# DeepMed-Lab-ECNU/BCP

Measured on AMD Instinct MI355X. Metric: training volumes/sec (LA 112x112x80 V-Net, BCP self-training step), higher is better.
Workload: dtype f32 (fp16x2 split operands); 1 GPU; LA 3D V-Net BCP self-train step, per-GPU batch 4 (2 labeled), 112x112x80 patches, SGD m0.9 wd1e-4, EMA 0.99 (BASELINE.json configs[1]); global_batch=4, parallelism=dp1

## Files before the change

bcp_amd/csrc/conv3.hip:

```cpp
#include "conv3_defs.h"
#include "../../include/bcp_hip.h"
#include <cstdlib>
#include <cstdio>

namespace bcp {

template <int KD, int TD, int TH, int TW, int NT, int WT>
__global__ __launch_bounds__(256) void k_conv3_mfma(const float* __restrict__ X, const float* __restrict__ Wp,
                                                    const float* __restrict__ bias, float* __restrict__ Y, ConvDims cd,
                                                    int accumulate, StatsArg st) {
  using TL = Tile<KD, TD, TH, TW>;
  constexpr int MT = TL::MT, T = TL::T, CT = NT * 16;
  constexpr int S = T / WT;
  static_assert(T % WT == 0, "WT must divide the tap count");
  constexpr int NBUF = (S > 1) ? 2 : 1;
  constexpr int WSTAGE4 = WT * 4 * CT;
  constexpr int NW4 = (WSTAGE4 + 255) / 256;
  constexpr int NACC = (MT * NT == 1) ? 2 : 1;

  HIP_DYNAMIC_SHARED(float4, smem4)
  float* smem = reinterpret_cast<float*>(smem4);
  float* Xs = smem;
  float* Ws = smem + TL::HV * XS;
  double* Ss = reinterpret_cast<double*>(Ws + NBUF * WSTAGE4 * 4);
// ... 781 lines not shown
    const bool twin = (d.dgrad & 0x800) != 0 && di > 0;
    d.dgrad &= 1;
    const int nb = d.N16 >> 4, k0 = (u / nb) * 16, n0 = (u % nb) * 16, T = d.T;
    const int row0 = d.dgrad ? k0 : n0, in0 = d.dgrad ? n0 : k0;
    for (int q = threadIdx.x; q < 256 * T; q += 256) {
      const int r = q / (16 * T), rem = q - r * 16 * T;
      const int in = rem / T, t = rem - in * T;
      float v = 0.f;
      if (row0 + r < d.Cout && in0 + in < d.Cin) v = d.w[((long long)(row0 + r) * d.Cin + in0 + in) * T + t];
      tile[q] = v;
    }
    __syncthreads();
    if (sec & 1)
    for (int q = threadIdx.x; q < 256 * T; q += 256) {
      const int k4 = q & 3, nn = (q >> 2) & 15, kq = (q >> 6) & 3, t = q >> 8;
      const int kk = kq * 4 + k4;
      const float v = d.dgrad ? tile[(kk * 16 + nn) * T + (T - 1 - t)] : tile[(nn * 16 + kk) * T + t];
      d.wp[(((long long)t * (d.K16 >> 2) + (k0 >> 2) + kq) * d.N16 + n0 + nn) * 4 + k4] = v;
    }
    {
      const int TP = (T + 1) / 2, ch = k0 >> 4;
      unsigned* wb = reinterpret_cast<unsigned*>(d.wp + (long long)T * d.K16 * d.N16);
      if (sec & 2)
      for (int q = threadIdx.x; q < TP * 16 * 16; q += 256) {
        const int j2 = q & 15, nn = (q >> 4) & 15, tp = q >> 8;
        const int t = 2 * tp + (j2 >> 3), kk = (j2 * 2) & 15;
        float v0 = 0.f, v1 = 0.f;
        if (t < T) {
          v0 = d.dgrad ? tile[(kk * 16 + nn) * T + (T - 1 - t)] : tile[(nn * 16 + kk) * T + t];
          v1 = d.dgrad ? tile[((kk + 1) * 16 + nn) * T + (T - 1 - t)] : tile[(nn * 16 + kk + 1) * T + t];
        }
        unsigned* o = wb + ((((((long long)ch * TP + tp) * 3) * d.N16 + n0 + nn) * 32 + j2 * 2) >> 1);
        const long long ps = ((long long)d.N16 * 32) >> 1;
        unsigned h = cvt_pk_bf16(v0, v1);
        o[0] = h;
        v0 -= __uint_as_float(h << 16); v1 -= __uint_as_float(h & 0xffff0000u);
        h = cvt_pk_bf16(v0, v1);
        o[ps] = h;
        v0 -= __uint_as_float(h << 16); v1 -= __uint_as_float(h & 0xffff0000u);
        o[2 * ps] = cvt_pk_bf16(v0, v1);
      }
      float* hdr = d.wp + pack_off_hdr(T, d.K16, d.N16);
      const float* hsrc = hdr;
      if (twin) { const PackDesc t = descs[di - 1]; hsrc = t.wp + pack_off_hdr(t.T, t.K16, t.N16); }
      float amax = 0.f;
#pragma unroll
      for (int b = 0; b < 16; ++b) amax = fmaxf(amax, hsrc[1 + b]);
      const float sc = f16_scale(amax);
      if (u == 0 && threadIdx.x == 0) hdr[0] = amax;
      unsigned* wh = reinterpret_cast<unsigned*>(d.wp + pack_off_f16(T, d.K16, d.N16));
      if (sec & 4)
      for (int q = threadIdx.x; q < TP * 16 * 16; q += 256) {
        const int j2 = q & 15, nn = (q >> 4) & 15, tp = q >> 8;
        const int t = 2 * tp + (j2 >> 3), kk = (j2 * 2) & 15;
        float v0 = 0.f, v1 = 0.f;
        if (t < T) {
          v0 = d.dgrad ? tile[(kk * 16 + nn) * T + (T - 1 - t)] : tile[(nn * 16 + kk) * T + t];
          v1 = d.dgrad ? tile[((kk + 1) * 16 + nn) * T + (T - 1 - t)] : tile[(nn * 16 + kk + 1) * T + t];
        }
        v0 *= sc; v1 *= sc;
        unsigned* o = wh + ((((((long long)ch * TP + tp) * 2) * d.N16 + n0 + nn) * 32 + j2 * 2) >> 1);
        const long long ps = ((long long)d.N16 * 32) >> 1;
        const unsigned h = cvt_pk_f16(v0, v1);
        o[0] = h;
        o[ps] = cvt_pk_f16(v0 - f16lo_to_f32(h), v1 - f16hi_to_f32(h));
      }
    }
    __syncthreads();
  }
}

struct C1Norm {
  const float* stats;
  const float* da;
  const float* c1c2;
  const uint8_t* elem_mask;
  float elem_scale;
  int act, G;
  float* amax;
  const unsigned long long* mask_seed;
  float p_keep;
};

template <int KD, int TD, int TH, int TW, int EPI = 0>
__global__ __launch_bounds__(256) void k_conv3_c1(const float* __restrict__ X, const float* __restrict__ w ,
                                                  const float* __restrict__ bias, float* __restrict__ Y, ConvDims cd, int n_tiles,
                                                  int tiles_per_block, StatsArg st, C1Norm nm) {
  using TL = Tile<KD, TD, TH, TW>;
  constexpr int T = TL::T, MT = TL::MT, KS = (T + 3) / 4;
  __shared__ __attribute__((aligned(16))) float Xs[TL::HV];
  __shared__ double Ss[4 * 16 * 2];
  __shared__ __attribute__((aligned(16))) float Ys[EPI == 5 ? TL::M * 16 : 4];
  static_assert(EPI != 5 || (TL::M == 256 && T <= 32 && MT == 4), "EPI 5: four waves x 64 voxels, two 16-tap MFMA row tiles");
  const int lane = threadIdx.x & 63, wave = threadIdx.x >> 6;
  const int li = lane & 15, lg = lane >> 4;
  int aoff[2] = {0, 0};
  f32x4 wacc[2] = {(f32x4){0.f, 0.f, 0.f, 0.f}, (f32x4){0.f, 0.f, 0.f, 0.f}};
  if (EPI == 5) {
#pragma unroll
    for (int tt = 0; tt < 2; ++tt) aoff[tt] = (tt * 16 + li < T) ? TL::tapoff(tt * 16 + li) : 0;
  }
  float wv[KS];
  int toff[KS];
#pragma unroll
  for (int ks = 0; ks < KS; ++ks) {
    const int tap = ks * 4 + lg;
    wv[ks] = tap < T ? w[li * T + tap] : 0.f;
    toff[ks] = tap < T ? TL::tapoff(tap) : 0;
  }
  float4 bv = make_float4(0.f, 0.f, 0.f, 0.f);
  if (bias) bv = ld4(bias + lg * 4);
  double s1[4] = {0, 0, 0, 0}, s2[4] = {0, 0, 0, 0};
  float amax_o = 0.f;
  unsigned mseed_lo = 0, mseed_hi = 0;
  if (EPI >= 2 && nm.mask_seed) { const unsigned long long s_ = *nm.mask_seed; mseed_lo = (unsigned)s_; mseed_hi = (unsigned)(s_ >> 32); }
  const bool has_mask = EPI >= 2 && (nm.elem_mask != nullptr || nm.mask_seed != nullptr);
  const int t_begin = blockIdx.x * tiles_per_block;
  int t_end = t_begin + tiles_per_block;
  if (t_end > n_tiles) t_end = n_tiles;
  float mu[4] = {0, 0, 0, 0}, rs[4] = {1, 1, 1, 1}, sc[4] = {1, 1, 1, 1}, sh[4] = {0, 0, 0, 0}, k1[4] = {0, 0, 0, 0}, k2[4] = {0, 0, 0, 0};
  if (EPI >= 2) {
    const int g = t_begin / st.tiles_per_group;
    const long long GC = (long long)nm.G * 16, o = (long long)g * 16 + lg * 4;
#pragma unroll
    for (int r = 0; r < 4; ++r) {
      mu[r] = nm.stats[o + r]; rs[r] = nm.stats[GC + o + r]; sc[r] = nm.stats[2 * GC + o + r]; sh[r] = nm.stats[3 * GC + o + r];
      if (EPI >= 4) { k1[r] = nm.c1c2[o + r]; k2[r] = nm.c1c2[GC + o + r]; }
    }
  }
  constexpr bool PRE = KD == 3;
  constexpr int NPRE = (TL::HV + 255) / 256;
  float pre[NPRE];
  auto fetch = [&](int tile) __attribute__((always_inline)) {
    int n, d0, h0, w0;
    tile_origin(cd, tile, TD, TH, TW, n, d0, h0, w0);
#pragma unroll
    for (int i = 0; i < NPRE; ++i) {
      const int q = threadIdx.x + i * 256;
      const int hw = q % TL::HW, hh = (q / TL::HW) % TL::HH, hd = q / (TL::HW * TL::HH);
      const int d = d0 - TL::PD + hd, h = h0 - 1 + hh, wq = w0 - 1 + hw;
      float v = 0.f;
      if (q < TL::HV && (unsigned)d < (unsigned)cd.D && (unsigned)h < (unsigned)cd.H && (unsigned)wq < (unsigned)cd.W)
        v = X[(((long long)n * cd.D + d) * cd.H + h) * cd.W + wq];
      pre[i] = v;
    }
  };
  if (PRE && t_begin < t_end) fetch(t_begin);
  for (int tile = t_begin; tile < t_end; ++tile) {
    int n, d0, h0, w0;
    tile_origin(cd, tile, TD, TH, TW, n, d0, h0, w0);
    if (tile > t_begin) __syncthreads();
    if (!PRE) fetch(tile);
#pragma unroll
    for (int i = 0; i < NPRE; ++i)
      if (threadIdx.x + i * 256 < TL::HV) Xs[threadIdx.x + i * 256] = pre[i];
    __syncthreads();
    if (PRE && tile + 1 < t_end) fetch(tile + 1);
    const bool full = d0 + TD <= cd.D && h0 + TH <= cd.H && w0 + TW <= cd.W;
#pragma unroll
    for (int mt = 0; mt < MT; ++mt) {
      const int m = (wave * MT + mt) * 16 + li;
      const int vo = TL::voff(m);
      const int tw = m % TW, th = (m / TW) % TH, td = m / (TW * TH);
      const int d = d0 + td, h = h0 + th, wq = w0 + tw;
      const bool ok = full || (d < cd.D && h < cd.H && wq < cd.W);
      const long long e = ((((long long)n * cd.D + d) * cd.H + h) * cd.W + wq) * 16 + lg * 4;
      float4 dav = make_float4(0.f, 0.f, 0.f, 0.f);
      uchar4 m4 = make_uchar4(1, 1, 1, 1);
      if (EPI >= 3 && ok) dav = ld4(nm.da + e);
      if (has_mask && ok) m4 = nm.mask_seed ? bern_keep4(e, mseed_lo, mseed_hi, nm.p_keep) : *reinterpret_cast<const uchar4*>(nm.elem_mask + e);
      f32x4 acc = (f32x4){0.f, 0.f, 0.f, 0.f};
#pragma unroll
      for (int ks = 0; ks < KS; ++ks) acc = __builtin_amdgcn_mfma_f32_16x16x4f32(wv[ks], Xs[vo + toff[ks]], acc, 0, 0, 0);
      float4 dyl = make_float4(0.f, 0.f, 0.f, 0.f);
      if (ok) {
        const float yv[4] = {acc[0] + bv.x, acc[1] + bv.y, acc[2] + bv.z, acc[3] + bv.w};
        if (EPI == 0) st4(Y + e, make_float4(yv[0], yv[1], yv[2], yv[3]));
        if (EPI <= 1) {
          if (st.partial) {
#pragma unroll
            for (int r = 0; r < 4; ++r) { s1[r] += (double)yv[r]; s2[r] += (double)yv[r] * (double)yv[r]; }
          }
        } else {
          const float ms[4] = {m4.x ? nm.elem_scale : 0.f, m4.y ? nm.elem_scale : 0.f, m4.z ? nm.elem_scale : 0.f, m4.w ? nm.elem_scale : 0.f};
          const float dd[4] = {dav.x, dav.y, dav.z, dav.w};
          float o[4];
#pragma unroll
          for (int r = 0; r < 4; ++r) {
            const float z = (yv[r] - mu[r]) * sc[r] + sh[r];
            if (EPI == 2) {
              o[r] = act_fwd(z, nm.act);
              if (has_mask) o[r] *= ms[r];
              const float t = fabsf(o[r]);
              amax_o = (t > amax_o || t != t) ? t : amax_o;
            } else {
              const float cs = has_mask ? ms[r] : 1.f;
              const float dz = dd[r] * cs * act_grad(z, nm.act);
              const float xh = (yv[r] - mu[r]) * rs[r];
              if (EPI == 3) { s1[r] += (double)dz; s2[r] += (double)dz * (double)xh; }
              else o[r] = sc[r] * (dz - k1[r] - xh * k2[r]);
            }
          }
          if (EPI == 2 || EPI == 4) st4(Y + e, make_float4(o[0], o[1], o[2], o[3]));
          if (EPI == 5) dyl = make_float4(o[0], o[1], o[2], o[3]);
        }
      }
      if (EPI == 5) st4(Ys + m * 16 + lg * 4, dyl);
    }
    if (EPI == 5) {
      __syncthreads();
#pragma unroll 4
      for (int ks = 0; ks < 16; ++ks) {
        const int v = wave * 64 + ks * 4 + lg;
        const int vo = TL::voff(v);
        const float b = Ys[v * 16 + li];
        wacc[0] = __builtin_amdgcn_mfma_f32_16x16x4f32(Xs[vo + aoff[0]], b, wacc[0], 0, 0, 0);
        wacc[1] = __builtin_amdgcn_mfma_f32_16x16x4f32(Xs[vo + aoff[1]], b, wacc[1], 0, 0, 0);
      }
    }
  }
  if (EPI == 5) {
    __syncthreads();
    float* red = Ys;
#pragma unroll
    for (int tt = 0; tt < 2; ++tt)
#pragma unroll
      for (int r = 0; r < 4; ++r) red[(wave * 32 + tt * 16 + lg * 4 + r) * 16 + li] = wacc[tt][r];
    __syncthreads();
    for (int o = threadIdx.x; o < T * 16; o += 256)
      Y[(long long)blockIdx.x * T * 16 + o] = (red[o] + red[512 + o]) + (red[1024 + o] + red[1536 + o]);
  }
  if (st.partial) {
#pragma unroll
    for (int r = 0; r < 4; ++r) {
      double a = s1[r], b = s2[r];
#pragma unroll
      for (int o = 1; o < 16; o <<= 1) { a += __shfl_xor(a, o); b += __shfl_xor(b, o); }
      if (li == 0) { Ss[(wave * 16 + lg * 4 + r) * 2] = a; Ss[(wave * 16 + lg * 4 + r) * 2 + 1] = b; }
    }
    __syncthreads();
    if (threadIdx.x < 16) {
      const int c = threadIdx.x;
      double a = 0.0, b = 0.0;
#pragma unroll
      for (int wv_ = 0; wv_ < 4; ++wv_) { a += Ss[(wv_ * 16 + c) * 2]; b += Ss[(wv_ * 16 + c) * 2 + 1]; }
      const int gg = t_begin / st.tiles_per_group, row = (t_begin % st.tiles_per_group) / tiles_per_block;
      double* dst = st.partial + (((long long)gg * st.rows + row) * 16 + c) * 2;
      dst[0] = a; dst[1] = b;
    }
  }
  if (EPI == 2 && nm.amax) { __syncthreads(); block_amax_publish(amax_o, nm.amax); }
}

template <int KD, int TD, int TH, int TW>
__global__ __launch_bounds__(256) void k_conv3_c1_wgrad(const float* __restrict__ X, const float* __restrict__ dY,
                                                        float* __restrict__ partial, ConvDims cd, int tiles_total,
                                                        int tiles_per_group) {
  using TL = Tile<KD, TD, TH, TW>;
  constexpr int T = TL::T, M = TL::M;
  static_assert(M == 256 && T <= 32, "four waves x 64 voxels, two 16-tap MFMA row tiles");
  constexpr int NXS = (TL::HV + 255) / 256;
  __shared__ __attribute__((aligned(16))) float Xs[TL::HV];
  __shared__ __attribute__((aligned(16))) float Ys[M * 16];
  const int lane = threadIdx.x & 63, wave = threadIdx.x >> 6;
  const int li = lane & 15, lg = lane >> 4;
  const int grp = blockIdx.x;
  int t_end = (grp + 1) * tiles_per_group;
  if (t_end > tiles_total) t_end = tiles_total;
  int tile = grp * tiles_per_group;
  if (tile >= t_end) return;

  int aoff[2];
#pragma unroll
  for (int tt = 0; tt < 2; ++tt) aoff[tt] = (tt * 16 + li < T) ? TL::tapoff(tt * 16 + li) : 0;
  f32x4 acc[2] = {(f32x4){0.f, 0.f, 0.f, 0.f}, (f32x4){0.f, 0.f, 0.f, 0.f}};

  float px[NXS];
  float4 py[4];
  auto fetch = [&](int tl) {
    int n, d0, h0, w0;
    tile_origin(cd, tl, TD, TH, TW, n, d0, h0, w0);
#pragma unroll
    for (int u = 0; u < NXS; ++u) {
      const int q = threadIdx.x + u * 256;
      float v = 0.f;
      if (q < TL::HV) {
        const int hw = q % TL::HW, hh = (q / TL::HW) % TL::HH, hd = q / (TL::HW * TL::HH);
        const int d = d0 - TL::PD + hd, h = h0 - 1 + hh, wq = w0 - 1 + hw;
        if ((unsigned)d < (unsigned)cd.D && (unsigned)h < (unsigned)cd.H && (unsigned)wq < (unsigned)cd.W)
          v = X[(((long long)n * cd.D + d) * cd.H + h) * cd.W + wq];
      }
      px[u] = v;
    }
#pragma unroll
    for (int u = 0; u < 4; ++u) {
      const int q = threadIdx.x + u * 256;
      const int m = q >> 2, c4 = q & 3;
      const int tw = m % TW, th = (m / TW) % TH, td = m / (TW * TH);
      const int d = d0 + td, h = h0 + th, wq = w0 + tw;
      float4 v = make_float4(0.f, 0.f, 0.f, 0.f);
      if (d < cd.D && h < cd.H && wq < cd.W) v = ld4(dY + ((((long long)n * cd.D + d) * cd.H + h) * cd.W + wq) * 16 + c4 * 4);
      py[u] = v;
    }
  };
  auto stash = [&]() {
#pragma unroll
    for (int u = 0; u < NXS; ++u) {
      const int q = threadIdx.x + u * 256;
      if (q < TL::HV) Xs[q] = px[u];
    }
#pragma unroll
    for (int u = 0; u < 4; ++u) st4(Ys + (threadIdx.x + u * 256) * 4, py[u]);
  };
// ... 534 lines not shown
    default: c1_launch<0>(KD, grid, s, x, w, bias, y, cd, tiles, tpb, st, nm); break;
  }
  return st.rows;
}

extern "C" int bcp_conv3_c1_fwd(const float* x, const float* w, const float* bias, float* y, int N, int D, int H, int W, int KD,
                                void* stream) {
  BCP_REQUIRE(x && w && y, "bcp_conv3_c1_fwd: null pointer");
  BCP_REQUIRE((KD == 1 && D == 1) || KD == 3, "bcp_conv3_c1_fwd: bad KD/D");
  BCP_REQUIRE(aligned16(y) && (!bias || aligned16(bias)), "bcp_conv3_c1_fwd: y / bias must be 16-B aligned");
  c1_fwd_impl(x, w, bias, y, N, D, H, W, KD, nullptr, 0, false, (hipStream_t)stream);
  BCP_CHECK_LAUNCH("bcp_conv3_c1_fwd");
  return BCP_OK;
}

extern "C" int bcp_conv3_c1_stat_rows(int N, int D, int H, int W, int KD, int groups) {
  if (groups < 1 || N < 1 || D < 1 || H < 1 || W < 1 || !((KD == 1 && D == 1) || KD == 3)) return 0;
  return c1_fwd_impl(nullptr, nullptr, nullptr, nullptr, N, D, H, W, KD, nullptr, groups, true, nullptr);
}

extern "C" int bcp_conv3_c1_fwd_stats(const float* x, const float* w, const float* bias, float* y, int N, int D, int H, int W, int KD,
                                      double* stat_partial, int groups, void* stream) {
  BCP_REQUIRE(x && w && y && stat_partial && groups >= 1, "bcp_conv3_c1_fwd_stats: null pointer / bad groups");
  BCP_REQUIRE((KD == 1 && D == 1) || KD == 3, "bcp_conv3_c1_fwd_stats: bad KD/D");
  BCP_REQUIRE(aligned16(y) && (!bias || aligned16(bias)), "bcp_conv3_c1_fwd_stats: y / bias must be 16-B aligned");
  const int rows = c1_fwd_impl(x, w, bias, y, N, D, H, W, KD, stat_partial, groups, false, (hipStream_t)stream);
  BCP_REQUIRE(rows > 0, "bcp_conv3_c1_fwd_stats: fused statistics unavailable (N %% groups != 0): check bcp_conv3_c1_stat_rows first");
  BCP_CHECK_LAUNCH("bcp_conv3_c1_fwd_stats");
  return BCP_OK;
}

namespace bcp {
void norm_fwd_finalize_launch(const double* partial, int nb, int G, int C, long long rows_per_group, const float* gamma, const float* beta,
                              float* running_mean, float* running_var, float momentum, float eps, float* stats, hipStream_t s, float* amax_clear_or_null);
void norm_bwd_finalize_launch(const double* partial, int nb, int G, int C, long long rows_per_group, float* dgamma, float* dbeta, int accumulate,
                              float* c1c2raw, hipStream_t s, float* amax_clear_or_null);
}

extern "C" size_t bcp_conv3_c1_norm_workspace_bytes(int N, int D, int H, int W, int KD, int groups) {
  const int rows = bcp_conv3_c1_stat_rows(N, D, H, W, KD, groups);
  return rows > 0 ? (size_t)groups * rows * 16 * 2 * sizeof(double) + (size_t)4 * groups * 16 * sizeof(float) : 0;
}

extern "C" int bcp_conv3_c1_norm_fwd(const float* x, const float* w, const float* bias, int N, int D, int H, int W, int KD, int groups,
                                     const float* gamma, const float* beta, float* running_mean, float* running_var, float momentum, float eps,
                                     int act, const uint8_t* elem_mask, float elem_scale, const unsigned long long* mask_seed, float mask_p_keep,
                                     float* stats, void* workspace, float* out, float* amax_out_or_null, void* stream) {
  BCP_REQUIRE(x && w && stats && workspace && out && groups >= 1, "bcp_conv3_c1_norm_fwd: null pointer / bad groups");
  BCP_REQUIRE((KD == 1 && D == 1) || KD == 3, "bcp_conv3_c1_norm_fwd: bad KD/D");
  BCP_REQUIRE(aligned16(out) && aligned16(stats) && (!bias || aligned16(bias)), "bcp_conv3_c1_norm_fwd: alignment");
  hipStream_t s = (hipStream_t)stream;
  double* partial = reinterpret_cast<double*>(workspace);
  const int rows = c1_fwd_impl(x, w, bias, nullptr, N, D, H, W, KD, partial, groups, false, s, 1);
  BCP_REQUIRE(rows > 0, "bcp_conv3_c1_norm_fwd: the groups must be whole samples (N %% groups == 0)");
  norm_fwd_finalize_launch(partial, rows, groups, 16, (long long)N / groups * D * H * W, gamma, beta, running_mean, running_var, momentum, eps, stats, s,
                           amax_out_or_null);
  const C1Norm nm{stats, nullptr, nullptr, elem_mask, elem_scale, act, groups, amax_out_or_null, mask_seed, mask_p_keep};
  c1_fwd_impl(x, w, bias, out, N, D, H, W, KD, nullptr, groups, false, s, 2, &nm);
  BCP_CHECK_LAUNCH("bcp_conv3_c1_norm_fwd");
  return BCP_OK;
}

extern "C" int bcp_conv3_c1_norm_bwd(const float* x, const float* w, const float* bias, const float* da, int N, int D, int H, int W, int KD,
                                     int groups, const float* stats, int act, const uint8_t* elem_mask, float elem_scale,
                                     const unsigned long long* mask_seed, float mask_p_keep, float* dgamma,
                                     float* dbeta, int accumulate, void* workspace, float* dy, void* stream) {
  BCP_REQUIRE(x && w && da && stats && workspace && dy && groups >= 1, "bcp_conv3_c1_norm_bwd: null pointer / bad groups");
  BCP_REQUIRE((KD == 1 && D == 1) || KD == 3, "bcp_conv3_c1_norm_bwd: bad KD/D");
  BCP_REQUIRE(aligned16(da) && aligned16(dy) && (!bias || aligned16(bias)), "bcp_conv3_c1_norm_bwd: alignment");
  BCP_REQUIRE((dgamma == nullptr) == (dbeta == nullptr), "bcp_conv3_c1_norm_bwd: dgamma and dbeta come together");
  hipStream_t s = (hipStream_t)stream;
  double* partial = reinterpret_cast<double*>(workspace);
  const int rows0 = bcp_conv3_c1_stat_rows(N, D, H, W, KD, groups);
  BCP_REQUIRE(rows0 > 0, "bcp_conv3_c1_norm_bwd: the groups must be whole samples (N %% groups == 0)");
  float* c1c2raw = reinterpret_cast<float*>(partial + (size_t)groups * rows0 * 16 * 2);
  C1Norm nm{stats, da, c1c2raw, elem_mask, elem_scale, act, groups, nullptr, mask_seed, mask_p_keep};
  const int rows = c1_fwd_impl(x, w, bias, nullptr, N, D, H, W, KD, partial, groups, false, s, 3, &nm);
  norm_bwd_finalize_launch(partial, rows, groups, 16, (long long)N / groups * D * H * W, dgamma, dbeta, accumulate, c1c2raw, s, nullptr);
  c1_fwd_impl(x, w, bias, dy, N, D, H, W, KD, nullptr, groups, false, s, 4, &nm);
  BCP_CHECK_LAUNCH("bcp_conv3_c1_norm_bwd");
  return BCP_OK;
}

extern "C" size_t bcp_conv3_c1_norm_bwd_wgrad_workspace_bytes(int N, int D, int H, int W, int KD, int groups) {
  const int rows = bcp_conv3_c1_stat_rows(N, D, H, W, KD, groups);
  if (rows <= 0) return 0;
  return bcp_conv3_c1_norm_workspace_bytes(N, D, H, W, KD, groups) + (size_t)groups * rows * (KD * 9) * 16 * sizeof(float);
}

extern "C" int bcp_conv3_c1_norm_bwd_wgrad(const float* x, const float* w, const float* bias, const float* da, int N, int D, int H, int W, int KD,
                                           int groups, const float* stats, int act, const uint8_t* elem_mask, float elem_scale,
                                           const unsigned long long* mask_seed, float mask_p_keep, float* dgamma, float* dbeta,
                                           int accumulate, void* workspace, float* dw, int dw_accumulate, void* stream) {
  BCP_REQUIRE(x && w && da && stats && workspace && dw && groups >= 1, "bcp_conv3_c1_norm_bwd_wgrad: null pointer / bad groups");
  BCP_REQUIRE((KD == 1 && D == 1) || KD == 3, "bcp_conv3_c1_norm_bwd_wgrad: bad KD/D");
  BCP_REQUIRE(aligned16(da) && (!bias || aligned16(bias)), "bcp_conv3_c1_norm_bwd_wgrad: alignment");
  BCP_REQUIRE((dgamma == nullptr) == (dbeta == nullptr), "bcp_conv3_c1_norm_bwd_wgrad: dgamma and dbeta come together");
  hipStream_t s = (hipStream_t)stream;
  double* partial = reinterpret_cast<double*>(workspace);
  const int rows0 = bcp_conv3_c1_stat_rows(N, D, H, W, KD, groups);
  BCP_REQUIRE(rows0 > 0, "bcp_conv3_c1_norm_bwd_wgrad: the groups must be whole samples (N %% groups == 0)");
  float* c1c2raw = reinterpret_cast<float*>(partial + (size_t)groups * rows0 * 16 * 2);
  float* wpart = c1c2raw + (size_t)4 * groups * 16;
  C1Norm nm{stats, da, c1c2raw, elem_mask, elem_scale, act, groups, nullptr, mask_seed, mask_p_keep};
  const int rows = c1_fwd_impl(x, w, bias, nullptr, N, D, H, W, KD, partial, groups, false, s, 3, &nm);
  norm_bwd_finalize_launch(partial, rows, groups, 16, (long long)N / groups * D * H * W, dgamma, dbeta, accumulate, c1c2raw, s, nullptr);
  c1_fwd_impl(x, w, bias, wpart, N, D, H, W, KD, nullptr, groups, false, s, 5, &nm);
  const int G = groups * rows, T = KD * 9;
  if (G >= 32 || options().wgrad_reduce_flat == 2)
    launch_reduce_deep(wpart, dw, G, T, 1, 16, 1, 16, dw_accumulate, s);
  else
    hipLaunchKernelGGL(k_wgrad_reduce, dim3(1, 1), dim3(256), 0, s, wpart, dw, G, T, 1, 16, 1, 16, dw_accumulate);
  BCP_CHECK_LAUNCH("bcp_conv3_c1_norm_bwd_wgrad");
  return BCP_OK;
}

extern "C" int bcp_conv3_c1_wgrad(const float* x, const float* dy, float* dw, int N, int D, int H, int W, int KD, int accumulate,
                                  void* workspace, void* stream) {
  BCP_REQUIRE(x && dy && dw && workspace, "bcp_conv3_c1_wgrad: null pointer");
  BCP_REQUIRE((KD == 1 && D == 1) || KD == 3, "bcp_conv3_c1_wgrad: bad KD/D");
  ConvDims cd;
  fill_dims(cd, N, D, H, W, 1, 16);
  float* ws = reinterpret_cast<float*>(workspace);
  int G;
  if (KD == 3) {
    cd.tiles_d = cdiv(D, 4); cd.tiles_h = cdiv(H, 4); cd.tiles_w = cdiv(W, 16);
    const int tiles = N * cd.tiles_d * cd.tiles_h * cd.tiles_w;
    const int g0 = tiles < 512 ? tiles : 512, tpg = cdiv(tiles, g0);
    G = cdiv(tiles, tpg);
    hipLaunchKernelGGL((k_conv3_c1_wgrad<3, 4, 4, 16>), dim3(G), dim3(256), 0, (hipStream_t)stream, x, dy, ws, cd, tiles, tpg);
  } else {
    cd.tiles_d = 1; cd.tiles_h = cdiv(H, 16); cd.tiles_w = cdiv(W, 16);
    const int tiles = N * cd.tiles_h * cd.tiles_w;
    const int g0 = tiles < 512 ? tiles : 512, tpg = cdiv(tiles, g0);
    G = cdiv(tiles, tpg);
    hipLaunchKernelGGL((k_conv3_c1_wgrad<1, 1, 16, 16>), dim3(G), dim3(256), 0, (hipStream_t)stream, x, dy, ws, cd, tiles, tpg);
  }
  const int T = KD * 9;
  if (G >= 32 || options().wgrad_reduce_flat == 2)
    launch_reduce_deep(ws, dw, G, T, 1, 16, 1, 16, accumulate, (hipStream_t)stream);
  else
    hipLaunchKernelGGL(k_wgrad_reduce, dim3(1, 1), dim3(256), 0, (hipStream_t)stream, ws, dw, G, T, 1, 16, 1, 16, accumulate);
  BCP_CHECK_LAUNCH("bcp_conv3_c1_wgrad");
  return BCP_OK;
}
```

bcp_amd/csrc/norm.hip:

```cpp
#include "common.h"
#include "../../include/bcp_hip.h"

namespace bcp {

struct NormEpilogue {
  const float* chan_scale;
  const uint8_t* elem_mask;
  float elem_scale;
  long long rows_per_sample;
  int act;
  const unsigned long long* mask_seed;
  float p_keep;
};
#define BCP_NORM_MASK_PROLOGUE(ep)                                                                                  \
  unsigned mseed_lo = 0, mseed_hi = 0;                                                                              \
  if ((ep).mask_seed) { const unsigned long long s_ = *(ep).mask_seed; mseed_lo = (unsigned)s_; mseed_hi = (unsigned)(s_ >> 32); } \
  const bool has_mask = (ep).elem_mask != nullptr || (ep).mask_seed != nullptr;
#define BCP_NORM_MASK4(ep, e) ((ep).mask_seed ? bern_keep4((e), mseed_lo, mseed_hi, (ep).p_keep) : *reinterpret_cast<const uchar4*>((ep).elem_mask + (e)))

struct SlabSrc { const float* slabs; int nslab; long long stride; const float* bias; float* sum_out; };

template <int MODE, bool SL = false>
__global__ __launch_bounds__(256) void k_col_partial(const float* __restrict__ y, const float* __restrict__ da,
                                                     const float* __restrict__ scale, const float* __restrict__ shift,
// ... 959 lines not shown
  do {                                                                                                                \
    const int rpp_ = (kOwnThreads / ((a_).cw / 4)) / (GS_);                                                             \
    const int P_ = (int)(((R_) + rpp_ - 1) / rpp_);                                                                   \
    const dim3 grid_((C_) / (a_).cw, (G_) / (GS_));                                                                        \
    if (P_ <= 1) hipLaunchKernelGGL((KERN<1>), grid_, dim3(kOwnThreads), 0, s_, a_, b_);                              \
    else if (P_ == 2) hipLaunchKernelGGL((KERN<2>), grid_, dim3(kOwnThreads), 0, s_, a_, b_);                         \
    else hipLaunchKernelGGL((KERN<4>), grid_, dim3(kOwnThreads), 0, s_, a_, b_);                                      \
  } while (0)

static inline bool fin_fused_ok(int nb, int C) { return options().norm_fuse_fin != 0 && nb >= 1 && nb <= kFinMaxRows && C >= 16 && C <= 256; }
static inline dim3 fin_grid(long long seg_rows, int nseg, int C, bool runner) {
  const int cw = C < kFinChunk ? C : kFinChunk, slots = 256 / (cw / 4);
  long long gx = (seg_rows + (long long)slots * 4 - 1) / ((long long)slots * 4);
  const long long cap = 1024 / ((long long)nseg * (C / cw)) < 1 ? 1 : 1024 / ((long long)nseg * (C / cw));
  if (gx > cap) gx = cap;
  return dim3((unsigned)(gx < 1 ? 1 : gx) + (runner ? 1u : 0u), (unsigned)nseg, (unsigned)(C / cw));
}

static inline bool skip_fin(long long rpg) { const int w = options().whatif; return (w & 1) || ((w & 2) && rpg <= 4096); }
static inline bool skip_app(long long rpg) { return ((options().whatif & 2) && rpg <= 4096) || ((options().whatif & 16) && rpg >= 100000); }
static inline bool skip_bstat(long long rpg) { return (options().whatif & 32) && rpg >= 100000; }
static inline int norm_blocks(long long rows_per_group, int C) {
  const int slots = 256 / (C / 4);
  long long nb = rows_per_group / ((long long)slots * 16);
  if (nb > 1024) nb = 1024;
  if (nb < 1) nb = 1;
  return (int)nb;
}

static inline int norm_blocks_slabs(long long rows_per_group, int C, int G, bool sizing = false ) {
  const int slots = 256 / (C / 4);
  long long nb = (rows_per_group + slots - 1) / slots;
  long long cap = G >= 256 ? 1 : 256 / G;
  if (!sizing && options().norm_fuse_fin != 0 && C <= 256 && cap > options().norm_fin_rows && options().norm_fin_rows > 0) cap = options().norm_fin_rows;
  if (nb > cap) nb = cap;
  const int plain = norm_blocks(rows_per_group, C);
  return (int)(nb < plain ? plain : nb);
}

static inline int apply_grid(long long nvec, int nseg) {
  const int vec = options().norm_apply_vec > 0 ? options().norm_apply_vec : 4, capw = options().norm_apply_cap > 0 ? options().norm_apply_cap : 2048;
  long long g = (nvec + 256 * vec - 1) / (256 * vec);
  const long long cap = capw / nseg < 1 ? 1 : capw / nseg;
  if (g > cap) g = cap;
  return (int)(g < 1 ? 1 : g);
}

struct Segs { long long seg_rows; int spg; int nbps; };
static inline Segs make_segs(int G, long long rows_per_group, int C, const NormEpilogue& ep, int nblocks = 0) {
  Segs sg{rows_per_group, 1, nblocks > 0 ? nblocks : norm_blocks(rows_per_group, C)};
  if (ep.chan_scale && ep.rows_per_sample < rows_per_group) {
    sg.seg_rows = ep.rows_per_sample;
    sg.spg = (int)(rows_per_group / ep.rows_per_sample);
    sg.nbps = sg.nbps / sg.spg < 1 ? 1 : sg.nbps / sg.spg;
  }
  return sg;
}
static constexpr int kMaxSamplesPerGroup = 64;

void norm_fwd_finalize_launch(const double* partial, int nb, int G, int C, long long rows_per_group, const float* gamma, const float* beta,
                              float* running_mean, float* running_var, float momentum, float eps, float* stats, hipStream_t s, float* amax_clear_or_null) {
  float *mean = stats, *rstd = stats + (long long)G * C, *scale = stats + 2LL * G * C, *shift = stats + 3LL * G * C, *var_unb = stats + 4LL * G * C;
  if (!skip_fin(rows_per_group)) hipLaunchKernelGGL(k_norm_finalize, dim3(G * (C / 16)), dim3(kFinalizeThreads), 0, s, partial, nb, G, C, rows_per_group, gamma, beta, running_mean,
                     running_var, momentum, eps, mean, rstd, scale, shift, var_unb, amax_clear_or_null);
  if (running_mean) hipLaunchKernelGGL(k_norm_running_only, dim3(1), dim3(256), 0, s, mean, var_unb, G, C, running_mean, running_var, momentum);
}

__global__ __launch_bounds__(256) void k_norm_bwd_params(const float* __restrict__ raw, int G, int C, float* __restrict__ dgamma,
                                                         float* __restrict__ dbeta, int accumulate) {
  for (int c = threadIdx.x; c < C; c += blockDim.x) {
    float gb = accumulate ? dbeta[c] : 0.f, gg = accumulate ? dgamma[c] : 0.f;
    for (int g = 0; g < G; ++g) { gb += raw[g * C + c]; gg += raw[(long long)G * C + g * C + c]; }
    dbeta[c] = gb;
    dgamma[c] = gg;
  }
}

void norm_bwd_finalize_launch(const double* partial, int nb, int G, int C, long long rows_per_group, float* dgamma, float* dbeta, int accumulate,
                              float* c1c2raw, hipStream_t s, float* amax_clear_or_null) {
  float *c1 = c1c2raw, *c2 = c1 + (long long)G * C, *raw = c2 + (long long)G * C;
  if (!skip_fin(rows_per_group)) hipLaunchKernelGGL(k_norm_bwd_finalize, dim3(G * (C / 16)), dim3(kFinalizeThreads), 0, s, partial, nb, G, C, rows_per_group, dgamma, dbeta,
                     accumulate, c1, c2, raw, amax_clear_or_null);
  if (dgamma) hipLaunchKernelGGL(k_norm_bwd_params, dim3(1), dim3(256), 0, s, raw, G, C, dgamma, dbeta, accumulate);
}

}

using namespace bcp;

extern "C" size_t bcp_norm_workspace_bytes(int G, long long rows_per_group, int C) {
  if (G < 1 || C < 16 || rows_per_group < 1) return 0;
  const int nbmax = rows_per_group <= 4096 ? norm_blocks_slabs(rows_per_group, C, G, true) : norm_blocks(rows_per_group, C);
  return (size_t)G * (nbmax + kMaxSamplesPerGroup) * C * 2 * sizeof(double) + (size_t)4 * G * C * sizeof(float);
}

static int check_norm_args(const char* fn, int G, long long rows_per_group, int C) {
  BCP_REQUIRE(G >= 1 && rows_per_group >= 1, "%s: bad extents", fn);
  BCP_REQUIRE(C >= 16 && C <= 1024 && (C & (C - 1)) == 0, "%s: C=%d unsupported (need a power of two in 16..1024)", fn, C);
  return BCP_OK;
}

extern "C" int bcp_norm_fwd(const float* y, int G, long long rows_per_group, int C, const float* gamma, const float* beta,
                            float* running_mean, float* running_var, float momentum, float eps, int act,
                            const float* chan_scale, long long rows_per_sample, const uint8_t* elem_mask, float elem_scale,
                            const unsigned long long* mask_seed , float mask_p_keep,
                            const float* residual, float* stats , void* workspace,
                            const double* partial_in, int nb_in, float* out, long long out_ld ,
                            float* amax_out , void* stream) {
  if (int rc = check_norm_args("bcp_norm_fwd", G, rows_per_group, C)) return rc;
  if (out_ld == 0) out_ld = C;
  BCP_REQUIRE(out_ld >= C && (out_ld & 3) == 0, "bcp_norm_fwd: out_ld=%lld (need a multiple of 4 >= C)", out_ld);
  BCP_REQUIRE(y && stats && workspace, "bcp_norm_fwd: null pointer");
  BCP_REQUIRE(aligned16(y) && (!out || aligned16(out)) && aligned16(stats), "bcp_norm_fwd: alignment");
  BCP_REQUIRE(out || !residual, "bcp_norm_fwd: statistics-only mode (out = NULL) takes no residual");
  hipStream_t s = (hipStream_t)stream;
  NormEpilogue ep{chan_scale, elem_mask, elem_scale, rows_per_sample > 0 ? rows_per_sample : rows_per_group, act, mask_seed, mask_p_keep};
  BCP_REQUIRE(!chan_scale || (rows_per_group % ep.rows_per_sample == 0 && rows_per_group / ep.rows_per_sample <= kMaxSamplesPerGroup),
              "bcp_norm_fwd: a group must hold 1..%d whole samples", kMaxSamplesPerGroup);
  const Segs sg = make_segs(G, rows_per_group, C, ep);
  const int nseg = G * sg.spg, nb = sg.nbps * sg.spg;
  double* partial = reinterpret_cast<double*>(workspace);
  float *mean = stats, *rstd = stats + (long long)G * C, *scale = stats + 2LL * G * C, *shift = stats + 3LL * G * C;
  float* var_unb = stats + 4LL * G * C;
  int own_cw = 0;
  if (const int GS = (out && !partial_in) ? own_gs(G, rows_per_group, C, running_mean != nullptr, own_cw) : 0) {
    const OwnCommon oc{y, nullptr, 0, 0, nullptr, nullptr, G, C, (int)rows_per_group, GS, own_cw, ep, amax_out};
    const OwnFwd of{gamma, beta, running_mean, running_var, momentum, eps, residual, stats, out, out_ld};
    BCP_OWN_LAUNCH(k_norm_own_fwd, rows_per_group, GS, G, C, s, oc, of);
    BCP_CHECK_LAUNCH("bcp_norm_fwd");
    return BCP_OK;
  }
  const bool fused = out && !partial_in && fin_fused_ok(nb, C);
  if (partial_in) {
    if (!skip_fin(rows_per_group)) hipLaunchKernelGGL(k_norm_finalize, dim3(G * (C / 16)), dim3(kFinalizeThreads), 0, s, partial_in, nb_in, G, C, rows_per_group, gamma, beta,
                       running_mean, running_var, momentum, eps, mean, rstd, scale, shift, var_unb, out ? amax_out : (float*)nullptr);
  } else {
    hipLaunchKernelGGL((k_col_partial<0>), dim3(sg.nbps, nseg), dim3(256), 0, s, y, (const float*)nullptr, (const float*)nullptr,
                       (const float*)nullptr, (const float*)nullptr, (const float*)nullptr, ep, sg.seg_rows, sg.spg, C, partial, SlabSrc{},
                       fused ? amax_out : (float*)nullptr);
    if (!fused && !skip_fin(rows_per_group)) hipLaunchKernelGGL(k_norm_finalize, dim3(G * (C / 16)), dim3(kFinalizeThreads), 0, s, partial, nb, G, C, rows_per_group, gamma, beta,
                       running_mean, running_var, momentum, eps, mean, rstd, scale, shift, var_unb, out ? amax_out : (float*)nullptr);
  }
  if (fused)
    hipLaunchKernelGGL(k_norm_apply_fin, fin_grid(sg.seg_rows, nseg, C, running_mean != nullptr), dim3(256), 0, s, y, residual, ep, sg.seg_rows, sg.spg, G, C, rows_per_group,
                       FinFwd{partial, nb, gamma, beta, running_mean, running_var, momentum, eps, stats}, out, amax_out, out_ld);
  else if (out && skip_app(rows_per_group)) {}
  else if (out)
    hipLaunchKernelGGL(k_norm_apply, dim3(apply_grid(sg.seg_rows * (C / 4), nseg), nseg), dim3(256), 0, s, y, scale, shift, mean, residual,
                       ep, sg.seg_rows, sg.spg, G, C, out, var_unb, running_mean, running_var, momentum, amax_out, (long long)(out_ld / 4));
  else if (running_mean)
    hipLaunchKernelGGL(k_norm_running_only, dim3(1), dim3(256), 0, s, mean, var_unb, G, C, running_mean, running_var, momentum);
  BCP_CHECK_LAUNCH("bcp_norm_fwd");
  return BCP_OK;
}

extern "C" int bcp_norm_bwd(const float* y, const float* da, int G, long long rows_per_group, int C, const float* stats,
                            int act, const float* chan_scale, long long rows_per_sample, const uint8_t* elem_mask,
                            float elem_scale, const unsigned long long* mask_seed, float mask_p_keep, float* dgamma, float* dbeta, int accumulate, void* workspace,
                            const double* partial_in, int nb_in, float* dy, float* amax_out , void* stream) {
  if (int rc = check_norm_args("bcp_norm_bwd", G, rows_per_group, C)) return rc;
  BCP_REQUIRE(y && da && stats && workspace && dy, "bcp_norm_bwd: null pointer");
  hipStream_t s = (hipStream_t)stream;
  NormEpilogue ep{chan_scale, elem_mask, elem_scale, rows_per_sample > 0 ? rows_per_sample : rows_per_group, act, mask_seed, mask_p_keep};
  BCP_REQUIRE(!chan_scale || (rows_per_group % ep.rows_per_sample == 0 && rows_per_group / ep.rows_per_sample <= kMaxSamplesPerGroup),
              "bcp_norm_bwd: a group must hold 1..%d whole samples", kMaxSamplesPerGroup);
  const Segs sg = make_segs(G, rows_per_group, C, ep);
// ... 131 lines not shown
```

Before: 838.7 volumes/s.

## Fuse c1 norm backward stats and weight-grad into one conv pass with algebraic combine

The norm-backward for the first 1-channel conv previously ran the conv twice: once to gather dz/xh statistics, then a finalize, then again to compute the weight gradient from the normalized dy. The new code makes a single pass that accumulates X^T·dz, X^T·xh and the per-tap input sums into per-block slabs. A new combine kernel reduces these and forms dW = scale·(X^T dz − k1·sum X − k2·X^T xh) algebraically, and it also writes dgamma/dbeta. This removes a full conv pass and a separate reduce launch, at the cost of doubled MFMA and LDS work in the fused epilogue, a larger slab workspace, and an occupancy hint of 4 for that variant.

```diff
diff --git a/bcp_amd/csrc/conv3.hip b/bcp_amd/csrc/conv3.hip
--- a/bcp_amd/csrc/conv3.hip
+++ b/bcp_amd/csrc/conv3.hip
@@ -887,8 +887,10 @@
   float p_keep;
 };
 
+constexpr int kC1Slab = 36;
+
 template <int KD, int TD, int TH, int TW, int EPI = 0>
-__global__ __launch_bounds__(256) void k_conv3_c1(const float* __restrict__ X, const float* __restrict__ w ,
+__global__ __launch_bounds__(256, EPI == 5 ? 4 : 1)  void k_conv3_c1(const float* __restrict__ X, const float* __restrict__ w ,
                                                   const float* __restrict__ bias, float* __restrict__ Y, ConvDims cd, int n_tiles,
                                                   int tiles_per_block, StatsArg st, C1Norm nm) {
   using TL = Tile<KD, TD, TH, TW>;
@@ -896,11 +898,16 @@
   __shared__ __attribute__((aligned(16))) float Xs[TL::HV];
   __shared__ double Ss[4 * 16 * 2];
   __shared__ __attribute__((aligned(16))) float Ys[EPI == 5 ? TL::M * 16 : 4];
+  __shared__ __attribute__((aligned(16))) float Zs[EPI == 5 ? TL::M * 16 : 4];
+  __shared__ float G0s[EPI == 5 ? 4 * 32 : 1];
   static_assert(EPI != 5 || (TL::M == 256 && T <= 32 && MT == 4), "EPI 5: four waves x 64 voxels, two 16-tap MFMA row tiles");
+  constexpr int NTT = EPI == 5 ? (T + 15) / 16 : 1;
   const int lane = threadIdx.x & 63, wave = threadIdx.x >> 6;
   const int li = lane & 15, lg = lane >> 4;
   int aoff[2] = {0, 0};
   f32x4 wacc[2] = {(f32x4){0.f, 0.f, 0.f, 0.f}, (f32x4){0.f, 0.f, 0.f, 0.f}};
+  f32x4 zacc[2] = {(f32x4){0.f, 0.f, 0.f, 0.f}, (f32x4){0.f, 0.f, 0.f, 0.f}};
+  float g0[2] = {0.f, 0.f};
   if (EPI == 5) {
 #pragma unroll
     for (int tt = 0; tt < 2; ++tt) aoff[tt] = (tt * 16 + li < T) ? TL::tapoff(tt * 16 + li) : 0;
@@ -930,7 +937,7 @@
 #pragma unroll
     for (int r = 0; r < 4; ++r) {
       mu[r] = nm.stats[o + r]; rs[r] = nm.stats[GC + o + r]; sc[r] = nm.stats[2 * GC + o + r]; sh[r] = nm.stats[3 * GC + o + r];
-      if (EPI >= 4) { k1[r] = nm.c1c2[o + r]; k2[r] = nm.c1c2[GC + o + r]; }
+      if (EPI == 4) { k1[r] = nm.c1c2[o + r]; k2[r] = nm.c1c2[GC + o + r]; }
     }
   }
   constexpr bool PRE = KD == 3;
@@ -977,7 +984,7 @@
       f32x4 acc = (f32x4){0.f, 0.f, 0.f, 0.f};
 #pragma unroll
       for (int ks = 0; ks < KS; ++ks) acc = __builtin_amdgcn_mfma_f32_16x16x4f32(wv[ks], Xs[vo + toff[ks]], acc, 0, 0, 0);
-      float4 dyl = make_float4(0.f, 0.f, 0.f, 0.f);
+      float4 dzl = make_float4(0.f, 0.f, 0.f, 0.f), xhl = dzl;
       if (ok) {
         const float yv[4] = {acc[0] + bv.x, acc[1] + bv.y, acc[2] + bv.z, acc[3] + bv.w};
         if (EPI == 0) st4(Y + e, make_float4(yv[0], yv[1], yv[2], yv[3]));
@@ -989,7 +996,7 @@
         } else {
           const float ms[4] = {m4.x ? nm.elem_scale : 0.f, m4.y ? nm.elem_scale : 0.f, m4.z ? nm.elem_scale : 0.f, m4.w ? nm.elem_scale : 0.f};
           const float dd[4] = {dav.x, dav.y, dav.z, dav.w};
-          float o[4];
+          float o[4], xo[4];
 #pragma unroll
           for (int r = 0; r < 4; ++r) {
             const float z = (yv[r] - mu[r]) * sc[r] + sh[r];
@@ -1002,15 +1009,16 @@
               const float cs = has_mask ? ms[r] : 1.f;
               const float dz = dd[r] * cs * act_grad(z, nm.act);
               const float xh = (yv[r] - mu[r]) * rs[r];
-              if (EPI == 3) { s1[r] += (double)dz; s2[r] += (double)dz * (double)xh; }
-              else o[r] = sc[r] * (dz - k1[r] - xh * k2[r]);
+              if (EPI == 3 || EPI == 5) { s1[r] += (double)dz; s2[r] += (double)dz * (double)xh; }
+              if (EPI == 4) o[r] = sc[r] * (dz - k1[r] - xh * k2[r]);
+              if (EPI == 5) { o[r] = dz; xo[r] = xh; }
             }
           }
           if (EPI == 2 || EPI == 4) st4(Y + e, make_float4(o[0], o[1], o[2], o[3]));
-          if (EPI == 5) dyl = make_float4(o[0], o[1], o[2], o[3]);
+          if (EPI == 5) { dzl = make_float4(o[0], o[1], o[2], o[3]); xhl = make_float4(xo[0], xo[1], xo[2], xo[3]); }
         }
       }
-      if (EPI == 5) st4(Ys + m * 16 + lg * 4, dyl);
+      if (EPI == 5) { st4(Ys + m * 16 + lg * 4, dzl); st4(Zs + m * 16 + lg * 4, xhl); }
     }
     if (EPI == 5) {
       __syncthreads();
@@ -1018,22 +1026,40 @@
       for (int ks = 0; ks < 16; ++ks) {
         const int v = wave * 64 + ks * 4 + lg;
         const int vo = TL::voff(v);
-        const float b = Ys[v * 16 + li];
-        wacc[0] = __builtin_amdgcn_mfma_f32_16x16x4f32(Xs[vo + aoff[0]], b, wacc[0], 0, 0, 0);
-        wacc[1] = __builtin_amdgcn_mfma_f32_16x16x4f32(Xs[vo + aoff[1]], b, wacc[1], 0, 0, 0);
+        const float b1 = Ys[v * 16 + li], b2 = Zs[v * 16 + li];
+        const bool in = full || (d0 + v / (TW * TH) < cd.D && h0 + (v / TW) % TH < cd.H && w0 + v % TW < cd.W);
+#pragma unroll
+        for (int tt = 0; tt < NTT; ++tt) {
+          const float a = Xs[vo + aoff[tt]];
+          wacc[tt] = __builtin_amdgcn_mfma_f32_16x16x4f32(a, b1, wacc[tt], 0, 0, 0);
+          zacc[tt] = __builtin_amdgcn_mfma_f32_16x16x4f32(a, b2, zacc[tt], 0, 0, 0);
+          g0[tt] += in ? a : 0.f;
+        }
       }
     }
   }
   if (EPI == 5) {
     __syncthreads();
-    float* red = Ys;
-#pragma unroll
-    for (int tt = 0; tt < 2; ++tt)
-#pragma unroll
-      for (int r = 0; r < 4; ++r) red[(wave * 32 + tt * 16 + lg * 4 + r) * 16 + li] = wacc[tt][r];
+    float *red1 = Ys, *red2 = Zs;
+#pragma unroll
+    for (int tt = 0; tt < NTT; ++tt) {
+#pragma unroll
+      for (int r = 0; r < 4; ++r) {
+        red1[(wave * 32 + tt * 16 + lg * 4 + r) * 16 + li] = wacc[tt][r];
+        red2[(wave * 32 + tt * 16 + lg * 4 + r) * 16 + li] = zacc[tt][r];
+      }
+      float g = g0[tt];
+      g += __shfl_xor(g, 16);
+      g += __shfl_xor(g, 32);
+      if (lg == 0) G0s[wave * 32 + tt * 16 + li] = g;
+    }
     __syncthreads();
-    for (int o = threadIdx.x; o < T * 16; o += 256)
-      Y[(long long)blockIdx.x * T * 16 + o] = (red[o] + red[512 + o]) + (red[1024 + o] + red[1536 + o]);
+    float* slab = Y + (long long)blockIdx.x * T * kC1Slab;
+    for (int o = threadIdx.x; o < T * 16; o += 256) {
+      slab[(o >> 4) * kC1Slab + (o & 15)] = (red1[o] + red1[512 + o]) + (red1[1024 + o] + red1[1536 + o]);
+      slab[(o >> 4) * kC1Slab + 16 + (o & 15)] = (red2[o] + red2[512 + o]) + (red2[1024 + o] + red2[1536 + o]);
+    }
+    if (threadIdx.x < T) slab[threadIdx.x * kC1Slab + 32] = (G0s[threadIdx.x] + G0s[32 + threadIdx.x]) + (G0s[64 + threadIdx.x] + G0s[96 + threadIdx.x]);
   }
   if (st.partial) {
 #pragma unroll
@@ -1734,10 +1760,15 @@
   return BCP_OK;
 }
 
+namespace bcp {
+void c1_bwd_combine_launch(const double* partial, int nb, int G, long long rows_per_group, const float* stats, const float* slabs, int T, int slab_ld,
+                           float* dgamma, float* dbeta, int accumulate, float* dw, int dw_accumulate, hipStream_t s);
+}
+
 extern "C" size_t bcp_conv3_c1_norm_bwd_wgrad_workspace_bytes(int N, int D, int H, int W, int KD, int groups) {
   const int rows = bcp_conv3_c1_stat_rows(N, D, H, W, KD, groups);
   if (rows <= 0) return 0;
-  return bcp_conv3_c1_norm_workspace_bytes(N, D, H, W, KD, groups) + (size_t)groups * rows * (KD * 9) * 16 * sizeof(float);
+  return (size_t)groups * rows * 16 * 2 * sizeof(double) + (size_t)groups * rows * (KD * 9) * kC1Slab * sizeof(float);
 }
 
 extern "C" int bcp_conv3_c1_norm_bwd_wgrad(const float* x, const float* w, const float* bias, const float* da, int N, int D, int H, int W, int KD,
@@ -1752,17 +1783,11 @@
   double* partial = reinterpret_cast<double*>(workspace);
   const int rows0 = bcp_conv3_c1_stat_rows(N, D, H, W, KD, groups);
   BCP_REQUIRE(rows0 > 0, "bcp_conv3_c1_norm_bwd_wgrad: the groups must be whole samples (N %% groups == 0)");
-  float* c1c2raw = reinterpret_cast<float*>(partial + (size_t)groups * rows0 * 16 * 2);
-  float* wpart = c1c2raw + (size_t)4 * groups * 16;
-  C1Norm nm{stats, da, c1c2raw, elem_mask, elem_scale, act, groups, nullptr, mask_seed, mask_p_keep};
-  const int rows = c1_fwd_impl(x, w, bias, nullptr, N, D, H, W, KD, partial, groups, false, s, 3, &nm);
-  norm_bwd_finalize_launch(partial, rows, groups, 16, (long long)N / groups * D * H * W, dgamma, dbeta, accumulate, c1c2raw, s, nullptr);
-  c1_fwd_impl(x, w, bias, wpart, N, D, H, W, KD, nullptr, groups, false, s, 5, &nm);
-  const int G = groups * rows, T = KD * 9;
-  if (G >= 32 || options().wgrad_reduce_flat == 2)
-    launch_reduce_deep(wpart, dw, G, T, 1, 16, 1, 16, dw_accumulate, s);
-  else
-    hipLaunchKernelGGL(k_wgrad_reduce, dim3(1, 1), dim3(256), 0, s, wpart, dw, G, T, 1, 16, 1, 16, dw_accumulate);
+  float* slabs = reinterpret_cast<float*>(partial + (size_t)groups * rows0 * 16 * 2);
+  C1Norm nm{stats, da, nullptr, elem_mask, elem_scale, act, groups, nullptr, mask_seed, mask_p_keep};
+  const int rows = c1_fwd_impl(x, w, bias, slabs, N, D, H, W, KD, partial, groups, false, s, 5, &nm);
+  c1_bwd_combine_launch(partial, rows, groups, (long long)N / groups * D * H * W, stats, slabs, KD * 9, kC1Slab, dgamma, dbeta, accumulate, dw,
+                        dw_accumulate, s);
   BCP_CHECK_LAUNCH("bcp_conv3_c1_norm_bwd_wgrad");
   return BCP_OK;
 }
diff --git a/bcp_amd/csrc/norm.hip b/bcp_amd/csrc/norm.hip
--- a/bcp_amd/csrc/norm.hip
+++ b/bcp_amd/csrc/norm.hip
@@ -1065,6 +1065,64 @@
   if (!skip_fin(rows_per_group)) hipLaunchKernelGGL(k_norm_bwd_finalize, dim3(G * (C / 16)), dim3(kFinalizeThreads), 0, s, partial, nb, G, C, rows_per_group, dgamma, dbeta,
                      accumulate, c1, c2, raw, amax_clear_or_null);
   if (dgamma) hipLaunchKernelGGL(k_norm_bwd_params, dim3(1), dim3(256), 0, s, raw, G, C, dgamma, dbeta, accumulate);
+}
+
+__global__ __launch_bounds__(kFinalizeThreads) void k_c1_bwd_combine(const double* __restrict__ partial, int nb, int G, long long rows_per_group,
+                                                                     const float* __restrict__ stats, const float* __restrict__ slabs, int T, int ld,
+                                                                     float* __restrict__ dgamma, float* __restrict__ dbeta, int accumulate,
+                                                                     float* __restrict__ dW, int dw_accumulate) {
+  constexpr int C = 16, NC = 33, SL = kFinalizeThreads / 36;
+  __shared__ double sred[SL][NC];
+  __shared__ double gs[NC];
+  const int c = threadIdx.x & 15;
+  double s1 = 0.0, s2 = 0.0;
+  if ((int)blockIdx.x == T) {
+    float gb = 0.f, gg = 0.f;
+    if (threadIdx.x < C && accumulate) { gb = dbeta[c]; gg = dgamma[c]; }
+    for (int g = 0; g < G; ++g)
+      if (reduce_partials(partial, nb, C, g, 0, s1, s2)) { gb += (float)s1; gg += (float)s2; }
+    if (threadIdx.x < C) { dbeta[c] = gb; dgamma[c] = gg; }
+    return;
+  }
+  const int tap = blockIdx.x;
+  const int col = threadIdx.x % 36, slot = threadIdx.x / 36;
+  const long long rs = (long long)T * ld;
+  double acc = 0.0;
+  for (int g = 0; g < G; ++g) {
+    const bool own = reduce_partials(partial, nb, C, g, 0, s1, s2);
+    double a0 = 0.0, a1 = 0.0, a2 = 0.0, a3 = 0.0;
+    if (col < NC && slot < SL) {
+      const float* p = slabs + ((long long)g * nb * T + tap) * ld + col;
+      int b = slot;
+      for (; b + 3 * SL < nb; b += 4 * SL) {
+        const float v0 = p[b * rs], v1 = p[(b + SL) * rs], v2 = p[(b + 2 * SL) * rs], v3 = p[(b + 3 * SL) * rs];
+        a0 += (double)v0; a1 += (double)v1; a2 += (double)v2; a3 += (double)v3;
+      }
+      for (; b < nb; b += SL) a0 += (double)p[b * rs];
+      sred[slot][col] = (a0 + a1) + (a2 + a3);
+    }
+    __syncthreads();
+    if (threadIdx.x < NC) {
+      double t = 0.0;
+      for (int k = 0; k < SL; ++k) t += sred[k][threadIdx.x];
+      gs[threadIdx.x] = t;
+    }
+    __syncthreads();
+    if (own) {
+      const double k1 = (double)(float)(s1 / (double)rows_per_group), k2 = (double)(float)(s2 / (double)rows_per_group);
+      acc += (double)stats[(2LL * G + g) * C + c] * (gs[c] - k1 * gs[32] - k2 * gs[16 + c]);
+    }
+  }
+  if (threadIdx.x < C) {
+    float* o = dW + (long long)c * T + tap;
+    *o = dw_accumulate ? (*o + (float)acc) : (float)acc;
+  }
+}
+
+void c1_bwd_combine_launch(const double* partial, int nb, int G, long long rows_per_group, const float* stats, const float* slabs, int T, int slab_ld,
+                           float* dgamma, float* dbeta, int accumulate, float* dw, int dw_accumulate, hipStream_t s) {
+  hipLaunchKernelGGL(k_c1_bwd_combine, dim3(T + (dgamma ? 1 : 0)), dim3(kFinalizeThreads), 0, s, partial, nb, G, rows_per_group, stats, slabs, T, slab_ld,
+                     dgamma, dbeta, accumulate, dw, dw_accumulate);
 }
 
 }
```

Result: no change. 842.3 volumes/s (median of 6 runs) (+0.4%).
